# lppllppl920/EndoscopyDepthEstimation-Pytorch

Hardware: AMD Instinct MI355X
Metric: train frame-pairs/sec at 256x320 bs=8 (higher is better)
Workload: dtype f32

## Files before the change

endoscopydepthestimation-pytorch_amd/csrc/conv_dma_kernels.h:

```cpp
#pragma once

#include "conv_kernels.h"

namespace endo {

static __device__ __attribute__((aligned(16))) float g_pad_consts[8] = {__builtin_nanf(""), __builtin_nanf(""), __builtin_nanf(""), __builtin_nanf(""),
                                                                  0.0f, 0.0f, 0.0f, 0.0f};

typedef const __attribute__((address_space(1))) void* gptr_t;
typedef __attribute__((address_space(3))) void* lptr_t;

template <int KS, int KC, int Q, int WX, int R, int NBUF, int VEC, int IN = IN_PLAIN>
struct ConvDmaSmem {
    using G = ConvGeom<KS, KC, WX, R, VEC>;
    static constexpr int kW = KS * KS * KC * 16 * Q;
    static constexpr int kUG = (G::kTileX / 2) * (G::kTileY / 2);
    static constexpr int kUI = kUG / 4;
    static constexpr int kUStride = ((kUG + kUI - 8 + 31) / 32) * 32 + 8;
    static constexpr int kChan = (IN == IN_UNPOOL) ? kUStride : G::kCS;
    static constexpr int kBuf = KC * kChan + kW;
    static constexpr int kTail = 4 * 16 * Q + 8 * 16 * Q;
    static size_t bytes(int bn_cap) { return sizeof(float) * (NBUF * kBuf + 3 * bn_cap + kTail); }
};

template <int KS, int KC, int Q, int IN, int EPI, int WX, int R, int NBUF, int MINW, int VEC, int XF, int EXP = 0, int PH = -1, int BF = 0>
__global__ void __launch_bounds__(kConvThreads, MINW) conv_dma_kernel(const ConvParams p0) {
    static_assert(BF == 0 || (PH < 0 && (KS == 3 || KS == 1) && (IN == IN_BNRELU || IN == IN_PLAIN || (IN == IN_UNPOOL && KS == 1))),
                  "bf16 operands: the ordinary 3x3 convolution and the 1x1 convolutions of the transition-down layers");
    static_assert(PH < 0 || (KS == 3 && (Q % 2) == 0 && IN == IN_PLAIN && EPI == EPI_FWD), "phase mode is the transition-up forward");
    static_assert(IN != IN_UNPOOL || (KS == 1 && R % 2 == 0), "UNPOOL is the transition-down data gradient (1x1)");
    static_assert(NBUF == 1 || NBUF == 2, "one or two LDS buffers");
    static_assert(VEC == 1 || (VEC == 4 && IN != IN_UPSAMPLE && IN != IN_UNPOOL && IN != IN_SUBPIX), "16-byte DMA needs contiguous sources");
    static_assert(IN != IN_SUBPIX || (KS == 3 && EPI == EPI_FWD && PH < 0), "sub-pixel input mode is the transition-up data gradient");
    using G = ConvGeom<KS, KC, WX, R, VEC>;
    using S = ConvDmaSmem<KS, KC, Q, WX, R, NBUF, VEC, IN>;
    constexpr int KK = KS * KS;
    constexpr int NB = 16 * Q;
    constexpr int kWElems = S::kW;
    constexpr int kWPre = (kWElems + kConvThreads - 1) / kConvThreads;
    constexpr bool kDgrad = (EPI == EPI_DGRAD_BN || EPI == EPI_DGRAD_SUMPOOL);
    constexpr int kPhW = 2 * 12 * 16 + 16;
    static_assert(PH < 0 || KC * kPhW <= kWElems, "the phase weights fit the ordinary weight buffer");
    constexpr int kSubW = 4 * 16 * Q + 16;

    extern __shared__ __attribute__((aligned(16))) float smem[];
    float* s_aux = smem + NBUF * S::kBuf;
    int grp, n;
    group_of(p0, blockIdx.z, grp, n);
    const ConvParams p = group_view(p0, grp);
    const int groups = p0.group_n > 0 ? gridDim.z / p0.group_n : 1;
    const bool first_of_group = blockIdx.x == 0 && blockIdx.y == 0 && n == 0;
    (void)groups; (void)first_of_group;
    const int cap = p.bn_cap;

    const int tid = threadIdx.x;
    const int lane = tid & 63;
    const int wave = __builtin_amdgcn_readfirstlane(tid >> 6);
    const int tile = (gridDim.x & 7) == 0 ? xcd_remap(blockIdx.x, gridDim.x) : blockIdx.x;
    const int x0 = (tile % p.tiles_x) * G::kTileX;
    const int y0 = (tile / p.tiles_x) * G::kTileY;
    const int ph = PH == 2 ? static_cast<int>(blockIdx.y) : PH;
    const int co_base = (p.ksplit > 0 || PH == 2) ? 0 : blockIdx.y * NB;

    if constexpr (IN == IN_BNRELU) {
// ... 4 lines not shown
            s_aux[cap + c] = mean;
            s_aux[2 * cap + c] = beta;
        }
        for (int c = p.cin + tid; c < ((p.cin + KC - 1) / KC) * KC; c += kConvThreads) {
            s_aux[c] = 0.f; s_aux[cap + c] = 0.f; s_aux[2 * cap + c] = 0.f;
        }
    }
    if constexpr (EPI == EPI_DGRAD_BN) {
        float* cst = s_aux + 3 * cap;
        if (tid < NB) {
            const int c = co_base + tid;
            float mean = 0.f, rstd = 0.f, scale = 0.f, beta = 0.f;
            if (c < p.cout) {
                mean = p.bn_saved[2 * c];
                rstd = p.bn_saved[2 * c + 1];
                scale = p.bn_gamma[c] * rstd;
                beta = p.bn_beta[c];
            }
            cst[4 * tid] = scale; cst[4 * tid + 1] = beta; cst[4 * tid + 2] = mean; cst[4 * tid + 3] = rstd;
        }
    }

    f32x4 acc[R][Q];
#pragma unroll
    for (int r = 0; r < R; ++r)
#pragma unroll
        for (int q = 0; q < Q; ++q) acc[r][q] = f32x4{0.f, 0.f, 0.f, 0.f};

    const int wx = (wave % WX) * 16;
    const int wy = (wave / WX) * R;
    const int li = lane & 15;
    const int lk = lane >> 4;

    int goff[G::kPos];
    unsigned pos_ok = 0;
#pragma unroll
    for (int k = 0; k < G::kPos; ++k) {
        const int e = tid + k * kConvThreads;
        goff[k] = 0;
        if (e < G::kUnits) {
            const int ry = e / (G::kCols / VEC);
            const int rx = (e - ry * (G::kCols / VEC)) * VEC;
            const int gy = y0 - G::kHalo + ry;
            const int gx = x0 - G::kLeft + rx;
            if (gy >= 0 && gy < p.h && gx >= 0 && gx < p.w) {
                pos_ok |= (1u << k);
                if constexpr (IN == IN_UPSAMPLE) goff[k] = (gy >> 1) * p.in_w + (gx >> 1);
                else if constexpr (IN == IN_SUBPIX) goff[k] = 2 * gy * p.in_w + 2 * gx;
                else goff[k] = gy * p.in_w + gx;
            }
        }
    }
    constexpr int kUSlots = (IN == IN_UNPOOL) ? (KC * S::kUStride + kConvThreads - 1) / kConvThreads : 1;
    int uoff[kUSlots];
    if constexpr (IN == IN_UNPOOL) {
        constexpr int PC = G::kTileX / 2;
        const int ph = p.h >> 1, pw = p.w >> 1;
#pragma unroll
        for (int k = 0; k < kUSlots; ++k) {
            const int e = tid + k * kConvThreads;
            const int u = e % S::kUStride;
            int off = -1;
            if (e < KC * S::kUStride) {
                if (u < S::kUG) {
                    const int gy = (y0 >> 1) + u / PC, gx = (x0 >> 1) + u % PC;
                    if (gy < ph && gx < pw) off = gy * p.in_w + gx;
                } else if (u < S::kUG + S::kUI) {
                    const int q = u - S::kUG;
                    const int gy = (y0 >> 1) + q / (PC / 4), gx = (x0 >> 1) + 4 * (q % (PC / 4));
                    if (gy < ph && gx < pw) off = gy * p.in_w + gx;
                }
            }
            uoff[k] = off;
        }
    }
    const float* in_n = p.in + n * p.in_ns;
    const float* pad_in = g_pad_consts + (IN == IN_BNRELU ? 0 : 4);
    const float* pad_zero = g_pad_consts + 4;
    const int nchunks_all = (p.cin + KC - 1) / KC;
    int chunk_begin = 0, nchunks = nchunks_all;
    ConvParams po = p;
    if (p.ksplit > 0) {
        const int per = (nchunks_all + p.ksplit - 1) / p.ksplit;
        chunk_begin = blockIdx.y * per;
        nchunks = min(nchunks_all, chunk_begin + per);
        po.out = p.out + blockIdx.y * p.split_stride;
    }

    auto issue_dma = [&](int chunk, int buf) {
        const int c_base = chunk * KC;
        float* s_in = smem + buf * S::kBuf;
        float* s_w = s_in + KC * S::kChan;
        if constexpr (IN == IN_UNPOOL) {
            const uint8_t* idx_n = p.in_idx + n * p.idx_ns;
#pragma unroll
            for (int k = 0; k < kUSlots; ++k) {
                const int e0 = k * kConvThreads + wave * 64;
                if (e0 < KC * S::kUStride) {
                    const int e = e0 + lane;
                    const int ch = c_base + e / S::kUStride;
                    const bool is_code = (e % S::kUStride) >= S::kUG;
                    const void* src = pad_zero;
                    if (uoff[k] >= 0 && ch < p.cin) {
                        const int64_t o = static_cast<int64_t>(ch) * p.in_cs + uoff[k];
                        src = is_code ? static_cast<const void*>(idx_n + o) : static_cast<const void*>(in_n + o);
                    }
                    if (e < KC * S::kUStride) __builtin_amdgcn_global_load_lds((gptr_t)src, (lptr_t)(s_in + e0), 4, 0, 0);
                }
            }
        }
        int sub_ph = 0;
        if constexpr (IN == IN_SUBPIX) sub_ph = c_base / p.sub_c;
#pragma unroll
        for (int c = 0; c < (IN == IN_UNPOOL ? 0 : KC); ++c) {
            const int ch = c_base + c;
            const float* plane = in_n + static_cast<int64_t>(ch) * p.in_cs;
            if constexpr (IN == IN_SUBPIX)
                plane = in_n + static_cast<int64_t>(ch - sub_ph * p.sub_c) * p.in_cs + (sub_ph >> 1) * p.in_w + (sub_ph & 1);
#pragma unroll
            for (int k = 0; k < G::kPos; ++k) {
                const int e0 = k * kConvThreads + wave * 64;
                if (e0 < G::kUnits) {
                    const bool ok = (ch < p.cin) && (pos_ok & (1u << k));
                    const float* src = ok ? plane + goff[k] : pad_in;
                    if (e0 + lane < G::kUnits) {
// ... 203 lines not shown
                        const float* a_base = s_in + (quad * 4 + lk) * G::kCS + wy * G::kCols + wx + li + G::kColOff;
                        const float* b_base = s_w + (quad * 4 + lk) * NB + li;
                        float sc = 1.f, mn = 0.f, bt = 0.f;
                        if constexpr (IN == IN_BNRELU && !kInPlace) {
                            const int ch = chunk * KC + quad * 4 + lk;
                            sc = s_aux[ch]; mn = s_aux[cap + ch]; bt = s_aux[2 * cap + ch];
                        }
#pragma unroll
                        for (int r = 0; r < R; ++r) {
                            const float v = a_base[r * G::kCols];
                            a[i][r] = (IN == IN_BNRELU && !kInPlace) ? __builtin_fmaxf(fmaf(v - mn, sc, bt), 0.f) : v;
                        }
#pragma unroll
                        for (int q = 0; q < Q; ++q) b[i][q] = b_base[q * 16];
                    } else {
#pragma unroll
                        for (int r = 0; r < R; ++r) a[i][r] = 0.f;
#pragma unroll
                        for (int q = 0; q < Q; ++q) b[i][q] = 0.f;
                    }
                }
                bf16x4_bits ap[R];
#pragma unroll
                for (int r = 0; r < R; ++r) ap[r] = pack_bf16x4(a[0][r], a[1][r], a[2][r], a[3][r]);
#pragma unroll
                for (int q = 0; q < Q; ++q) {
                    const bf16x4_bits bp = pack_bf16x4(b[0][q], b[1][q], b[2][q], b[3][q]);
#pragma unroll
                    for (int r = 0; r < R; ++r) acc[r][q] = __builtin_amdgcn_mfma_f32_16x16x16bf16_1k(ap[r], bp, acc[r][q], 0, 0, 0);
                }
            }
            return;
        }
#pragma unroll
        for (int quad = 0; quad < KC / 4; ++quad) {
            const float* a_base = s_in + (quad * 4 + lk) * G::kCS + wy * G::kCols + wx + li + G::kColOff;
            const float* b_base = s_w + (quad * 4 + lk) * NB + li;
            float sc = 1.f, mn = 0.f, bt = 0.f;
            if constexpr (IN == IN_BNRELU && !kInPlace) {
                const int ch = chunk * KC + quad * 4 + lk;
                sc = s_aux[ch]; mn = s_aux[cap + ch]; bt = s_aux[2 * cap + ch];
            }
#pragma unroll
            for (int dx = 0; dx < KS; ++dx) {
                float a[R + KS - 1];
                if constexpr (BF != 0) {
#pragma unroll
                    for (int r = 0; r < R + 2; ++r) {
                        const float v = a_base[r * G::kCols + dx];
                        a[r] = (IN == IN_BNRELU && !kInPlace) ? __builtin_fmaxf(fmaf(v - mn, sc, bt), 0.f) : v;
                    }
                    bf16x4_bits ap[R];
#pragma unroll
                    for (int r = 0; r < R; ++r) ap[r] = pack_bf16x4(a[r], a[r + 1], a[r + 2], 0.f);
#pragma unroll
                    for (int q = 0; q < Q; ++q) {
                        const bf16x4_bits bp = pack_bf16x4(b_base[(0 * KS + dx) * KC * NB + q * 16], b_base[(1 * KS + dx) * KC * NB + q * 16],
                                                           b_base[(2 * KS + dx) * KC * NB + q * 16], 0.f);
#pragma unroll
                        for (int r = 0; r < R; ++r) acc[r][q] = __builtin_amdgcn_mfma_f32_16x16x16bf16_1k(ap[r], bp, acc[r][q], 0, 0, 0);
                    }
                    continue;
                }
                if constexpr (IN == IN_BNRELU && !kInPlace && !(EXP & 2)) {
                    typedef float f32x2 __attribute__((ext_vector_type(2)));
                    constexpr int NR = R + KS - 1;
// ... 27 lines not shown
                            const int tyi = dy - (sub_alpha == 0 ? 1 : 0), txi = dx - (sub_beta == 0 ? 1 : 0);
                            b = s_w[(quad * 4 + lk) * kSubW + (tyi * 2 + txi) * NB + q * 16 + li];
                        } else if constexpr (PH >= 0) {
                            const int slot = dx == 0 ? q : (dx == 1 ? Q / 2 + q : Q / 2 + Q + (q - Q / 2));
                            b = s_w[(quad * 4 + lk) * kPhW + ((dy - ph) * 2 * Q + slot) * 16 + li];
                        } else {
                            b = b_base[(dy * KS + dx) * KC * NB + q * 16];
                        }
#pragma unroll
                        for (int r = 0; r < R; ++r)
                            acc[r][q] = __builtin_amdgcn_mfma_f32_16x16x4f32(a[r + dy], b, acc[r][q], 0, 0, 0);
                    }
                }
            }
        }
    };

    issue_dma(chunk_begin, 0);
    if constexpr (kInPlace) {
        __syncthreads();
        asm volatile("s_waitcnt vmcnt(0)" ::: "memory");
        transform_own(chunk_begin, 0);
        __syncthreads();
        for (int chunk = chunk_begin; chunk < nchunks; ++chunk) {
            const int b = (chunk - chunk_begin) & 1;
            if (chunk + 1 < nchunks) issue_dma(chunk + 1, b ^ 1);
            compute(chunk, b);
            if (chunk + 1 < nchunks) {
                asm volatile("s_waitcnt vmcnt(0)" ::: "memory");
                transform_own(chunk + 1, b ^ 1);
            }
            __syncthreads();
        }
    } else {
        for (int chunk = chunk_begin; chunk < nchunks; ++chunk) {
            const int b = (chunk - chunk_begin) % NBUF;
            if (!(EXP & 4) || chunk == chunk_begin) asm volatile("s_waitcnt vmcnt(0)" ::: "memory");
            __syncthreads();
            if (NBUF == 2 && chunk + 1 < nchunks && !(EXP & 1)) issue_dma(chunk + 1, b ^ 1);
            compute(chunk, b);
            if (NBUF == 1 && chunk + 1 < nchunks) {
                __syncthreads();
                issue_dma(chunk + 1, 0);
            }
        }
    }

    if constexpr (EPI == EPI_DGRAD_BN) {
        if (use_pre) {
            const float* cst = s_aux + 3 * cap;
            float* s_red = s_aux + 3 * cap + 4 * NB;
            const int px = x0 + wx + 4 * lk;
#pragma unroll
            for (int q = 0; q < Q; ++q) {
                const int jloc = q * 16 + li;
                const int co = co_base + jloc;
                const float scale = cst[4 * jloc], beta = cst[4 * jloc + 1], mean = cst[4 * jloc + 2], rstd = cst[4 * jloc + 3];
                float s1 = 0.f, s2 = 0.f;
#pragma unroll
                for (int r = 0; r < R; ++r) {
                    const int y = y0 + wy + r;
                    if (co < p.cout && y < p.h && px + 3 < p.w) {
                        f32x4 o = dpre[r][q];
#pragma unroll
                        for (int e = 0; e < 4; ++e) {
                            const float xc = xpre[r][q][e] - mean;
// ... 107 lines not shown
```

endoscopydepthestimation-pytorch_amd/csrc/net.hip:

```cpp
#include <new>
#include <vector>

#include "dgrad_kernels.h"
#include "dgrad_block_kernels.h"
#include "dgrad_newmap_kernels.h"
#include "td_dgrad_kernels.h"
#include "td_fwd_kernels.h"
#include "wgrad_taps_kernels.h"
#include "wgrad1x1_kernels.h"
#include "wgrad_nsplit_kernels.h"
#include "wgrad_x3_kernels.h"
#include "wgrad_f34_kernels.h"
#include "wgrad_subpix_kernels.h"
#include "wino_fwd_kernels.h"
#include "wino4_fwd_kernels.h"
#include "dgrad_wino_kernels.h"
#include "dgrad_wino3_kernels.h"


namespace endo {

int run_dgrad_wino3_nl4(const DgradBlockParams& p, const float* const* u, hipStream_t stream);
bool dgrad_wino3p_applies(const DgradBlockParams& p);
int run_dgrad_wino3p_nl4(const DgradBlockParams& p, const float* const* u, int blocks, double* fw_parts, int* blocks_used, hipStream_t stream);
// ... 451 lines not shown
        const int stride = gridDim.y * blockDim.x * 4;
        for (int i = (blockIdx.y * blockDim.x + threadIdx.x) * 4; i < plane; i += stride) {
            const f32x4 gv = *reinterpret_cast<const f32x4*>(gp + i);
            const f32x4 pv = *reinterpret_cast<const f32x4*>(pp + i);
            f32x4 uv = {1.f, 1.f, 1.f, 1.f};
            if (c < cin) uv = *reinterpret_cast<const f32x4*>(up + i);
            part += gv[0] * sign_of(pv[0]) * uv[0] + gv[1] * sign_of(pv[1]) * uv[1];
            part2 += gv[2] * sign_of(pv[2]) * uv[2] + gv[3] * sign_of(pv[3]) * uv[3];
        }
    } else {
        for (int i = blockIdx.y * blockDim.x + threadIdx.x; i < plane; i += gridDim.y * blockDim.x)
            part += gp[i] * sign_of(pp[i]) * (c < cin ? up[i] : 1.f);
    }
    const int lane = threadIdx.x & 63, wave = threadIdx.x >> 6;
    double v = wave_sum(static_cast<double>(part + part2));
    if (lane == 0) scratch[wave] = v;
    __syncthreads();
    if (threadIdx.x == 0) {
        const float t = static_cast<float>(scratch[0] + scratch[1] + scratch[2] + scratch[3]);
        if (c < cin) atomicAdd(gw + c, t); else atomicAdd(gb, t);
    }
}

__global__ void __launch_bounds__(64) final_w_reduce_kernel(const double* __restrict__ parts, int nblocks, int count, float* __restrict__ gw) {
    const int c = blockIdx.x;
    double t = 0.0;
    for (int b = threadIdx.x; b < nblocks; b += 64) t += parts[static_cast<int64_t>(b) * count + c];
    t = wave_sum(t);
    if (threadIdx.x == 0) atomicAdd(gw + c, static_cast<float>(t));
}

constexpr int kBlocks = 2 * kLevels + 1, kDense = kBlocks * kLayers;

enum class DenseFwd { Wino4, Wino2_32x16, Wino2_32x8, SplitK, Direct32x8, Direct16x8, DirectAuto };
struct FwdPlan {
    struct Dense {
        DenseFwd form;
        int stages;
        int ksplit;
        bool chunk_weights;
    } dense[kDense];
    bool bf16;
    bool wino4_weights;
    bool fuse_final;
    bool td_persistent[kLevels];
    bool tu_subpix[kLevels];
};

enum class NewMap { Bf16, Persistent, Vec16, Dword };
enum class BasePass { Block8, Block8Bf16, Wino3, Wino3Persistent, Wino8 };
enum class DenseWgrad { F34, X3, NSplit, Taps, Direct };
enum class TdDgrad { Persistent, Runs128, Dma, Staged };
enum class TuWgrad { Subpix, Taps, Direct };
enum class TuDgrad { Subpix32x8, Subpix16x8, Subpix16x4, Plain };
enum class FirstWgrad { F34Prep, F34, Taps, Direct };
struct BwdPlan {
    struct Block {
        bool fused;
        NewMap newmap[kLayers];
        BasePass base;
        bool wino3_layout;
    } block[kBlocks];
    DenseWgrad wgrad[kDense];
    bool td_wgrad_dma[kLevels];
    TdDgrad td_dgrad[kLevels];
    TuWgrad tu_wgrad[kLevels];
    TuDgrad tu_dgrad[kLevels];
    int overlap;
    bool bf16_wgrad, bf16_dgrad;
    int f34_blocks;
    bool dgrad_weights;
    bool use_virt;
    bool virt_base;
// ... 60 lines not shown
    p.cin = cin;
}

static void fill_out(const Ctx& c, ConvParams& p, float* base, int level, int oc0, int cout) {
    const auto& lv = c.net->lv[level];
    p.out = base + oc0 * lv.plane;
    p.out_ns = lv.t * lv.plane;
    p.out_cs = static_cast<int>(lv.plane);
    p.out_w = lv.w;
    p.cout = cout;
}

static void fill_grid(const Ctx& c, ConvParams& p, int level) {
    const auto& lv = c.net->lv[level];
    p.n = c.nt(); p.h = lv.h; p.w = lv.w;
    p.group_n = c.net->n; p.gs = c.net->gs; p.in_gs = c.net->gs; p.out_gs = c.net->gs;
}

static double conv_flops(const endo_net* net, int level, int cin, int cout, int ks) {
    return 2.0 * net->n * net->groups * net->lv[level].plane * cin * cout * ks * ks;
}

static void default_options(int (&opt)[ENDO_OPT_COUNT]) {
    opt[ENDO_OPT_WINO_FWD] = 5;
    opt[ENDO_OPT_WINO_DGRAD] = 3;
    opt[ENDO_OPT_DGRAD_VEC] = 2;
    opt[ENDO_OPT_WINO_MIN_TILES] = 1024;
    opt[ENDO_OPT_MFMA_BF16] = 0;
    opt[ENDO_OPT_WGRAD_OVERLAP] = 1;
    opt[ENDO_OPT_MFMA_X3] = 0;
    opt[ENDO_OPT_WGRAD_F34] = 1;
    opt[ENDO_OPT_FINAL_VIRTUAL] = 1;
    opt[ENDO_OPT_TD_PERSIST] = 3;
}
static int bf16_mask(const int* opt) { const int v = opt[ENDO_OPT_MFMA_BF16]; return v == 1 ? 7 : (v >> 1); }

struct DenseBlock { int level, ic0, c0; const BnP* bn; const ConvP* cv; bool base_overwrite; };
static DenseBlock dense_block(int b) {
    const Table& tb = table();
    if (b < kLevels) return {b, 48, down_in(b), tb.down_bn[b], tb.down_conv[b], false};
    if (b == kLevels) return {kLevels, 0, 288, tb.bott_bn, tb.bott_conv, true};
    const int i = b - kLevels - 1, l = kLevels - 1 - i;
    return {l, 0, 96 + down_in(l), tb.up_bn[i], tb.up_conv[i], l > 0};
}
static long tile_count(const Ctx& c, int level, int tx, int ty) {
    const auto& lv = c.net->lv[level];
    return static_cast<long>((lv.w + tx - 1) / tx) * ((lv.h + ty - 1) / ty) * c.nt();
}

static ConvParams dense_fwd_params(const Ctx& c, const DenseBlock& k, int j, DenseFwd form) {
    const ConvP& cv = k.cv[j];
    const int oc0 = k.ic0 + k.c0 + kGrowth * j;
    ConvParams p{};
    fill_grid(c, p, k.level);
    fill_in(c, p, c.act(k.level), k.level, k.ic0, cv.cin);
    fill_bn_in(c, p, k.bn[j], k.level, k.ic0);
    p.wgt = c.params + cv.w; p.bias = c.params + cv.b; p.w_cout = cv.cout; p.w_cin = cv.cin;
    fill_out(c, p, c.act(k.level), k.level, oc0, cv.cout);
    p.out_sums = c.out_sums(k.level, oc0);
    if (form == DenseFwd::Wino4) p.wgt = c.tape + c.net->wino4_off + cv.u / kWinoUStride * kW4UStride;
    if (form == DenseFwd::Wino2_32x16 || form == DenseFwd::Wino2_32x8) p.wgt = c.tape + c.net->wino_off + cv.u;
    return p;
}

static ConvParams td_fwd_params(const Ctx& c, int level) {
    const BnP& b = table().td_bn[level];
    const ConvP& cv = table().td_conv[level];
    const int next = level + 1;
    const int oc0 = next < kLevels ? 48 : 0;
    ConvParams p{};
    fill_grid(c, p, level);
    fill_in(c, p, c.act(level), level, 48, cv.cin);
    fill_bn_in(c, p, b, level, 48);
    p.wgt = c.params + cv.w; p.bias = c.params + cv.b; p.w_cout = cv.cout; p.w_cin = cv.cin;
    fill_out(c, p, c.act(next), next, oc0, cv.cout);
    p.out_idx = c.idx(level);
    p.idx_ns = static_cast<int64_t>(cv.cout) * c.net->lv[next].plane;
    p.out_sums = c.out_sums(next, oc0);
    return p;
}

static FwdPlan plan_fwd(const Ctx& c) {
    const int* opt = c.net->opt;
    const int mode = opt[ENDO_OPT_WINO_FWD];
    const long min_tiles = opt[ENDO_OPT_WINO_MIN_TILES];
    FwdPlan pl{};
    pl.bf16 = (bf16_mask(opt) & 2) != 0;
    pl.wino4_weights = !pl.bf16 && mode == 5;
    for (int b = 0; b < kBlocks; ++b) {
        const DenseBlock k = dense_block(b);
        const long t64x16 = tile_count(c, k.level, 64, 16), t32x16 = tile_count(c, k.level, 32, 16), t32x8 = tile_count(c, k.level, 32, 8);
        const long t16x16 = tile_count(c, k.level, 16, 16), t16x8 = tile_count(c, k.level, 16, 8);
        const bool big = t32x16 >= min_tiles, small = t32x8 >= (min_tiles * 3) / 4;
        const bool wino4_tiles = mode == 5 && !pl.bf16 && 2 * t64x16 >= min_tiles;
        const bool wino2_tiles = mode != 0 && !pl.bf16 && (big || small);
        for (int j = 0; j < kLayers; ++j) {
            FwdPlan::Dense& d = pl.dense[b * kLayers + j];
            const int nchunks = (k.cv[j].cin + 15) / 16;
            d.chunk_weights = !pl.bf16 && !wino4_tiles && !wino2_tiles;
            d.stages = mode == 4 ? 4 : (mode == 3 ? 3 : 2);
            if (wino4_tiles && wino4_fwd_ok(dense_fwd_params(c, k, j, DenseFwd::Wino4))) {
                d.form = DenseFwd::Wino4;
            } else if (wino2_tiles && wino_fwd_ok(dense_fwd_params(c, k, j, DenseFwd::Wino2_32x16))) {
                d.form = big ? DenseFwd::Wino2_32x16 : DenseFwd::Wino2_32x8;
            } else if (t32x16 < 512 && t16x16 < 384 && t16x8 < 512 && nchunks >= 4) {
                int want = static_cast<int>(((t16x8 < 256 ? 512 : 768) + t16x8 - 1) / t16x8);
                if (want > nchunks) want = nchunks;
                const int per = (nchunks + want - 1) / want;
                d.form = DenseFwd::SplitK;
                d.ksplit = (nchunks + per - 1) / per;
            } else {
                d.form = (t32x16 < 1024 && t32x8 >= 1024) ? DenseFwd::Direct32x8
                       : (t32x16 < 1024 && t16x8 >= 768) ? DenseFwd::Direct16x8 : DenseFwd::DirectAuto;
            }
        }
    }
    pl.fuse_final = opt[ENDO_OPT_FINAL_VIRTUAL] && pl.dense[kDense - 1].form == DenseFwd::Wino4;
    for (int l = 0; l < kLevels; ++l) {
        pl.td_persistent[l] = (opt[ENDO_OPT_TD_PERSIST] & 2) && !pl.bf16 && c.training && td_fwd_ok(td_fwd_params(c, l));
        const ConvP& tu = table().tu_conv[kLevels - 1 - l];
        pl.tu_subpix[l] = c.net->lv[l + 1].w % 4 == 0 && tu.cout == kNew && tu.cin % 4 == 0;
    }
    return pl;
}

static int dense_fwd(const Ctx& c, int b, int j) {
    const DenseBlock k = dense_block(b);
    const FwdPlan::Dense& d = c.fwd->dense[b * kLayers + j];
    const ConvP& cv = k.cv[j];
    const auto& lv = c.net->lv[k.level];
    const int oc0 = k.ic0 + k.c0 + kGrowth * j;
    ConvParams p = dense_fwd_params(c, k, j, d.form);
    ProfScope prof(kProfConv3x3Dense, c.stream, conv_flops(c.net, k.level, cv.cin, cv.cout, 3),
                   4.0 * c.nt() * lv.plane * (cv.cin + cv.cout));
    const float* chunk_weights = d.chunk_weights ? c.tape + c.net->wino_off + cv.u : nullptr;
    const bool bf16 = c.fwd->bf16;
    switch (d.form) {
        case DenseFwd::Wino4:
            if (c.fwd->fuse_final && b == kBlocks - 1 && j == kLayers - 1) { p.fin_w = c.params + table().final_.w + k.ic0; p.fin_out = c.tape + c.net->pre_off; }
            return launch_wino4_fwd(p, c.stream);
        case DenseFwd::Wino2_32x16:
            return d.stages == 4 ? launch_wino_fwd<2, 4, 2, 4>(p, c.stream) : d.stages == 3 ? launch_wino_fwd<2, 4, 2, 3>(p, c.stream) : launch_wino_fwd<2, 4, 2, 2>(p, c.stream);
        case DenseFwd::Wino2_32x8:
            return d.stages == 4 ? launch_wino_fwd<1, 4, 3, 4>(p, c.stream) : d.stages == 3 ? launch_wino_fwd<1, 4, 3, 3>(p, c.stream) : launch_wino_fwd<1, 4, 3, 2>(p, c.stream);
        case DenseFwd::SplitK: {
            float* partial = c.tape + c.net->partial_off;
            p.ksplit = d.ksplit;
            p.split_stride = static_cast<int64_t>(c.net->n) * cv.cout * lv.plane;
            p.out = partial; p.out_ns = static_cast<int64_t>(cv.cout) * lv.plane;
            p.bias = nullptr; p.out_sums = nullptr;
            p.wgt_chunks = chunk_weights;
            int rc = bf16 ? launch_conv_dma<3, 16, 1, IN_BNRELU, EPI_FWD, 1, 2, 2, 1, 1>(p, c.stream)
                          : launch_conv_dma<3, 16, 1, IN_BNRELU, EPI_FWD, 1, 2, 2, 1>(p, c.stream);
            if (rc) return rc;
            int bx = static_cast<int>((lv.plane + 255) / 256);
            bx = bx > 8 ? 8 : bx;
            finalize_partial_kernel<<<dim3(bx, cv.cout, c.nt()), 256, 0, c.stream>>>(
                partial, p.split_stride, d.ksplit, p.out_ns, static_cast<int>(lv.plane), c.params + cv.b, c.act(k.level) + oc0 * lv.plane,
                lv.t * lv.plane, c.out_sums(k.level, oc0), c.net->n, c.net->gs);
            ENDO_LAUNCH_CHECK();
            return 0;
        }
        case DenseFwd::Direct32x8:
            return bf16 ? launch_conv_dma<3, 4, 1, IN_BNRELU, EPI_FWD, 2, 4, 2, 1, 1>(p, c.stream) : launch_conv_dma<3, 4, 1, IN_BNRELU, EPI_FWD, 2, 4, 2, 1>(p, c.stream);
        case DenseFwd::Direct16x8:
            return bf16 ? launch_conv_dma<3, 8, 1, IN_BNRELU, EPI_FWD, 1, 2, 2, 1, 1>(p, c.stream) : launch_conv_dma<3, 8, 1, IN_BNRELU, EPI_FWD, 1, 2, 2, 1>(p, c.stream);
        case DenseFwd::DirectAuto:
            if (bf16) return launch_conv_dma_auto<3, 4, 1, IN_BNRELU, EPI_FWD, 8, 2, 1, 1>(p, c.stream);
            p.wgt_chunks = chunk_weights;
            return launch_conv_dma_auto<3, 4, 1, IN_BNRELU, EPI_FWD, 8, 2, 1>(p, c.stream);
    }
    return ENDO_E_BADARG;
}

static int td_fwd(const Ctx& c, int level) {
    const ConvP& cv = table().td_conv[level];
    const ConvParams p = td_fwd_params(c, level);
    ProfScope prof(kProfConv1x1Pool, c.stream, conv_flops(c.net, level, cv.cin, cv.cout, 1),
                   4.0 * c.nt() * c.net->lv[level].plane * (cv.cin + cv.cout / 4.0));
    if (c.fwd->td_persistent[level]) return launch_td_fwd(p, device_cu_count(), c.stream);
    if (c.fwd->bf16) return launch_conv_dma_auto<1, 8, 3, IN_BNRELU, EPI_FWD_POOL, 4, 2, 1, 1>(p, c.stream);
    return launch_conv_dma_auto<1, 8, 3, IN_BNRELU, EPI_FWD_POOL, 4>(p, c.stream);
}

static int tu_fwd(const Ctx& c, int level, int src_level, int src_c0, const ConvP& cv) {
    ProfScope prof(kProfConv3x3Up, c.stream, conv_flops(c.net, level, cv.cin, cv.cout, 3),
                   4.0 * c.nt() * c.net->lv[level].plane * (cv.cin / 4.0 + cv.cout));
    if (c.fwd->tu_subpix[level]) {
        float* w3 = c.tape + c.net->partial_off;
        tu_phase_weights_kernel<<<(2 * cv.cin * 384 + 255) / 256, 256, 0, c.stream>>>(c.params + cv.w, cv.cout, cv.cin, w3);
        ENDO_LAUNCH_CHECK();
        ConvParams p{};
        fill_grid(c, p, src_level);
        fill_in(c, p, c.act(src_level), src_level, src_c0, cv.cin);
        p.wgt = w3; p.w_cout = 2 * cv.cout; p.w_cin = cv.cin;
// ... 567 lines not shown
    if (bn_index < 0 || bn_index >= static_cast<int>(tb.bn_order.size()) || which < 0 || which > 1) return -1;
    return tb.bn_order[bn_index]->run + which * tb.bn_order[bn_index]->c;
}
extern "C" int endo_net_level_channels(int level) { return (level < 0 || level > kLevels) ? -1 : level_channels(level); }
extern "C" int64_t endo_net_act_offset(const endo_net* net, int level) { return (!net || level < 0 || level > kLevels) ? -1 : net->lv[level].act; }

extern "C" int64_t endo_net_tape_offset(const endo_net* net, int what, int index) {
    if (!net) return -1;
    const Table& tb = table();
    switch (what) {
        case ENDO_TAPE_PRE: return net->pre_off;
        case ENDO_TAPE_BN_SAVED:
            if (index < 0 || index >= static_cast<int>(tb.bn_order.size())) return -1;
            return net->saved_off + 2 * tb.bn_order[index]->saved;
        case ENDO_TAPE_POOL:
            if (index < 0 || index >= kLevels) return -1;
            return net->idx_off[index];
        default: return -1;
    }
}

extern "C" int endo_net_fwd(endo_net* net, const float* params, float* bn_running, const float* x, float* out, float* tape,
                            int training, void* stream_) {
    if (!net || !params || !bn_running || !x || !out || !tape) return ENDO_E_BADARG;
    const Table& tb = table();
    Ctx c{net, params, bn_running, tape, nullptr, nullptr, training, static_cast<hipStream_t>(stream_)};
    const FwdPlan plan = plan_fwd(c);
    c.fwd = &plan;
    for (int g = 0; g < net->groups; ++g)
        ENDO_CHECK(hipMemsetAsync(reinterpret_cast<char*>(tape + g * net->gs) + net->sums_off, 0, net->sums_bytes, c.stream));
    if (!plan.bf16) {
        ProfScope prof(kProfSmall, c.stream, 0.0, 4.0 * (tb.wino_floats + tb.wino_floats * 9 / 16));
        WinoWeightTable wt = tb.wino;
        for (int l = 0; l < wt.layers; ++l) wt.mode[l] = plan.dense[l].chunk_weights ? 1 : 0;
        wino_fwd_weights_kernel<<<(wt.start[wt.layers] + 255) / 256, 256, 0, c.stream>>>(wt, params, tape + net->wino_off);
        ENDO_LAUNCH_CHECK();
        if (plan.wino4_weights) wino4_fwd_weights_kernel<<<(tb.wino4.start[tb.wino4.layers] + 255) / 256, 256, 0, c.stream>>>(tb.wino4, params, tape + net->wino4_off);
        ENDO_LAUNCH_CHECK();
    }
    int rc;
    {
        ConvParams p{};
        fill_grid(c, p, 0);
        p.in = x; p.in_ns = 3 * net->lv[0].plane; p.in_cs = static_cast<int>(net->lv[0].plane); p.in_w = net->w; p.cin = 3;
        p.in_gs = net->n * p.in_ns;
        p.wgt = params + tb.first.w; p.bias = params + tb.first.b; p.w_cout = kFirst; p.w_cin = 3;
        fill_out(c, p, c.act(0), 0, 48, kFirst);
        p.out_sums = c.out_sums(0, 48);
        ProfScope prof(kProfConvFirst, c.stream, conv_flops(net, 0, 3, kFirst, 3), 4.0 * c.nt() * net->lv[0].plane * (3 + kFirst));
        rc = launch_conv_dma_auto<3, 4, 3, IN_PLAIN, EPI_FWD>(p, c.stream);
        if (rc) return rc;
    }
    for (int b = 0; b < kBlocks; ++b) {
        if (b > kLevels) {
            const int i = b - kLevels - 1, l = kLevels - 1 - i;
            rc = tu_fwd(c, l, l + 1, (i == 0) ? 288 : 96 + down_in(l + 1), tb.tu_conv[i]);
            if (rc) return rc;
        }
        for (int j = 0; j < kLayers; ++j) {
            rc = dense_fwd(c, b, j);
            if (rc) return rc;
        }
        if (b < kLevels) {
            rc = td_fwd(c, b);
            if (rc) return rc;
        }
    }
// ... 118 lines not shown
```

endoscopydepthestimation-pytorch_amd/csrc/wino_fwd_kernels.h:

```cpp
#pragma once

#include "conv_dma_kernels.h"

namespace endo {

constexpr int kWinoUStride = 16 * 16 + 16;
constexpr int kWinoMaxLayers = 48;

struct WinoWeightTable {
    int layers;
    int start[kWinoMaxLayers + 1];
    int cin[kWinoMaxLayers];
    int cout[kWinoMaxLayers];
    int64_t w_off[kWinoMaxLayers];
    int64_t u_off[kWinoMaxLayers];
    int mode[kWinoMaxLayers];
};
constexpr int kDenseChunkFloats = 9 * 16 * 16;

__global__ void __launch_bounds__(256) wino_fwd_weights_kernel(const WinoWeightTable t, const float* __restrict__ params, float* __restrict__ u) {
    const int total = t.start[t.layers];
    for (int item = blockIdx.x * blockDim.x + threadIdx.x; item < total; item += gridDim.x * blockDim.x) {
        int l = 0;
        while (item >= t.start[l + 1]) ++l;
        const int e = item - t.start[l];
        const int ci = e >> 4, j = e & 15;
        float g[3][3];
#pragma unroll
        for (int a = 0; a < 3; ++a)
#pragma unroll
            for (int b = 0; b < 3; ++b) g[a][b] = 0.f;
        if (j < t.cout[l]) {
            const float* src = params + t.w_off[l] + (static_cast<int64_t>(j) * t.cin[l] + ci) * 9;
#pragma unroll
            for (int a = 0; a < 3; ++a)
#pragma unroll
                for (int b = 0; b < 3; ++b) g[a][b] = src[a * 3 + b];
        }
        if (t.mode[l] == 1) {
            float* dst = u + t.u_off[l] + static_cast<int64_t>(ci >> 4) * kDenseChunkFloats + (ci & 15) * 16 + j;
#pragma unroll
            for (int tap = 0; tap < 9; ++tap) dst[tap * 256] = g[tap / 3][tap % 3];
            if (ci == t.cin[l] - 1)
                for (int cz = (ci & 15) + 1; cz < 16; ++cz)
#pragma unroll
                    for (int tap = 0; tap < 9; ++tap) dst[tap * 256 + (cz - (ci & 15)) * 16] = 0.f;
            continue;
        }
        float h[4][3];
#pragma unroll
        for (int b = 0; b < 3; ++b) {
            h[0][b] = g[0][b];
            h[1][b] = 0.5f * (g[0][b] + g[1][b] + g[2][b]);
            h[2][b] = 0.5f * (g[0][b] - g[1][b] + g[2][b]);
            h[3][b] = g[2][b];
        }
        float* dst = u + t.u_off[l] + static_cast<int64_t>(ci) * kWinoUStride + j;
#pragma unroll
        for (int a = 0; a < 4; ++a) {
            dst[(4 * a + 0) * 16] = h[a][0];
            dst[(4 * a + 1) * 16] = 0.5f * (h[a][0] + h[a][1] + h[a][2]);
            dst[(4 * a + 2) * 16] = 0.5f * (h[a][0] - h[a][1] + h[a][2]);
            dst[(4 * a + 3) * 16] = h[a][2];
        }
        if (j == 0) {
#pragma unroll
            for (int k = 0; k < 16; ++k) dst[256 + k] = 0.f;
        }
    }
}

template <int R, int KC, int NS = 2>
struct WinoFwdGeom {
    static constexpr int kTileX = 32;
    static constexpr int kTileY = 8 * R;
    static constexpr int kLeft = 4;
    static constexpr int kCols = kTileX + 2 * kLeft;
    static constexpr int kRows = kTileY + 2;
    static constexpr int kPlane = kRows * kCols;
// ... 256 lines not shown
```

endoscopydepthestimation-pytorch_amd/models.py:

```python

import ctypes

import torch
from torch import nn

from . import _lib

GROWTH = 12
LAYERS = 4
FIRST = 48
LEVELS = 5


class ConvParams(nn.Module):

    def __init__(self, cin, cout, k):
        super().__init__()
        self.weight = nn.Parameter(torch.empty(cout, cin, k, k))
        self.bias = nn.Parameter(torch.zeros(cout))
        nn.init.kaiming_uniform_(self.weight, a=5 ** 0.5)


class FusedBatchNorm2d(nn.Module):

# ... 200 lines not shown
        if self._flat_grad is None or self._flat_grad.device != self._flat.device:
            if not create:
                return
            self._flat_grad_full = torch.zeros(self._flat.numel() + 1, dtype=torch.float32, device=self._flat.device)
            self._flat_grad = self._flat_grad_full[:self._flat.numel()]
            for p, off in zip(self._params, self._offsets):
                p.grad = self._flat_grad[off:off + p.numel()].view(p.shape)
            return
        base = self._flat_grad.data_ptr()
        intact = True
        for p, off in zip(self._params, self._offsets):
            g = p.grad
            if g is None or g.data_ptr() != base + 4 * off:
                intact = False
                break
        if not intact:
            self._flat_grad.zero_()
            for p, off in zip(self._params, self._offsets):
                p.grad = self._flat_grad[off:off + p.numel()].view(p.shape)

    def _handle(self, n, h, w, groups=1):
        key = (n, h, w, groups)
        if key not in self._handles:
            lib = _lib.load()
            if lib.endo_net_param_floats() != self._flat.numel():
                raise RuntimeError("parameter packing mismatch between Python and libendo_hip.so")
            hnd = ctypes.c_void_p()
            _lib.check(lib.endo_net_create_grouped(ctypes.byref(hnd), n, h, w, groups), "endo_net_create_grouped(%d,%d,%d,%d)" % key)
            for option_id, value in getattr(self, "_kernel_options", {}).items():
                lib.endo_net_set_option(hnd, option_id, value)
            self._handles[key] = (hnd, int(lib.endo_net_tape_floats(hnd)), int(lib.endo_net_gradws_floats(hnd)))
        return self._handles[key]

    _OPTION_DEFAULTS = {0: 5, 1: 3, 2: 2, 3: 1024, 4: 0, 5: 1, 6: 0, 7: 1, 8: 1, 9: 3}

    def set_kernel_option(self, option_id, value):
        option_id, value = int(option_id), int(value)
        if option_id not in self._OPTION_DEFAULTS:
            raise ValueError("unknown kernel option %d" % option_id)
        options = self.__dict__.setdefault("_kernel_options", {})
        old = options.get(option_id, self._OPTION_DEFAULTS[option_id])
        options[option_id] = value
        lib = _lib.load()
        for key, (hnd, _, _) in self._handles.items():
            if key[0] in ("bf16", "fp16"):
                continue
            rc = lib.endo_net_set_option(hnd, option_id, value)
            if rc < 0:
                raise RuntimeError("endo_net_set_option(%d, %d) failed: %d" % (option_id, value, rc))
        return old

    def kernel_option(self, option_id):
        return self.__dict__.get("_kernel_options", {}).get(int(option_id), self._OPTION_DEFAULTS[int(option_id)])

    def __del__(self):
        try:
            lib = _lib.load()
            for key, (hnd, _, _) in self._handles.items():
                {"bf16": lib.endo_net16_destroy, "fp16": lib.endo_net16h_destroy}.get(key[0], lib.endo_net_destroy)(hnd)
            self._handles = {}
        except Exception:
            pass

    def __getstate__(self):
        state = dict(self.__dict__)
        for key in ("_handles", "_gradws"):
            state[key] = {}
# ... 316 lines not shown
```

include/endo_hip.h:

```cpp
#ifndef ENDO_HIP_H
#define ENDO_HIP_H

#include <stdint.h>

#ifdef __cplusplus
extern "C" {
#endif

#define ENDO_E_BADARG (-1)
#define ENDO_E_UNSUPPORTED (-2)

#define ENDO_ABI_VERSION 6
int endo_abi_version(void);
const char* endo_error_string(int code);

int endo_depth_scale_fwd(const float* pred, const float* sparse_depth, const float* sparse_mask,
                         float* scaled, float* ratio, double* stats,
                         int n, int hw, float eps, void* stream);
int endo_depth_scale_bwd(const float* grad_scaled, const float* grad_ratio,
                         const float* pred, const float* sparse_depth, const double* stats,
                         float* grad_pred, double* work,
                         int n, int hw, float eps, void* stream);

int endo_flow_from_depth_fwd(const float* depth, const float* mask, const float* t, const float* R,
// ... 48 lines not shown
                   const float* sparse_flows_1, const float* sparse_flows_2,
                   const float* sparse_flow_masks_1, const float* sparse_flow_masks_2,
                   const float* t_1_wrt_2, const float* r_1_wrt_2, const float* t_2_wrt_1, const float* r_2_wrt_1,
                   const float* intrinsics, float sfl_weight, float dcl_weight, float eps,
                   float* losses, float* grad_pred_1, float* grad_pred_2, float* workspace,
                   int n, int h, int w, void* stream);
int endo_loss_head_planes(int n, int h, int w, int64_t* offsets);

int64_t endo_warp_consistency_workspace_floats(int n, int h, int w);
int64_t endo_warp_consistency_bytes(int n, int h, int w);
int endo_warp_consistency(const float* depth_1, const float* depth_2, const float* boundaries, const float* t_1_wrt_2,
                          const float* r_1_wrt_2, const float* t_2_wrt_1, const float* r_2_wrt_1, const float* intrinsics,
                          float dcl_weight, float eps, float* loss, float* grad_depth_1, float* grad_depth_2,
                          float* workspace, int n, int h, int w, void* stream);


int endo_mask_mul(const float* a, const float* mask, float* out, int n, int c, int hw, void* stream);

typedef struct endo_net endo_net;

int endo_net_create(endo_net** out, int n, int h, int w);
int endo_net_create_grouped(endo_net** out, int n, int h, int w, int groups);
int endo_net_groups(const endo_net* net);
#define ENDO_OPT_WINO_FWD 0
#define ENDO_OPT_WINO_DGRAD 1
#define ENDO_OPT_DGRAD_VEC 2
#define ENDO_OPT_WINO_MIN_TILES 3
#define ENDO_OPT_MFMA_BF16 4
#define ENDO_OPT_WGRAD_OVERLAP 5
#define ENDO_OPT_MFMA_X3 6
#define ENDO_OPT_WGRAD_F34 7
#define ENDO_OPT_FINAL_VIRTUAL 8
#define ENDO_OPT_TD_PERSIST 9
#define ENDO_OPT_COUNT 10
int endo_net_set_option(endo_net* net, int option_id, int value);
int endo_net_get_option(const endo_net* net, int option_id);
int64_t endo_net_group_stride(const endo_net* net);
void endo_net_destroy(endo_net* net);
int64_t endo_net_param_floats(void);
int64_t endo_net_bn_floats(void);
int64_t endo_net_tape_floats(const endo_net* net);
int64_t endo_net_gradws_floats(const endo_net* net);
int64_t endo_net_param_offset(int index);
int64_t endo_net_bn_offset(int bn_index, int which );

int endo_net_fwd(endo_net* net, const float* params, float* bn_running, const float* x, float* out,
                 float* tape, int training, void* stream);
int endo_net_bwd(endo_net* net, const float* params, const float* x, const float* tape,
                 const float* grad_out, float* grads, float* gradws, int training, void* stream);
int endo_net_level_channels(int level);
int64_t endo_net_act_offset(const endo_net* net, int level);
#define ENDO_TAPE_PRE 0
#define ENDO_TAPE_BN_SAVED 1
#define ENDO_TAPE_POOL 2
int64_t endo_net_tape_offset(const endo_net* net, int what, int index);

int endo_sgd_clip_step(float* params, float* grads, float* momentum, double* norm_out,
                       int64_t count, float lr, float mu, float max_norm, float grad_scale,
                       int first_step, const float* skip_flag, void* stream);

int endo_sparse_scatter(const double* points, int n_points, const double* projections, const double* extrinsics,
                        const float* visibility, const float* clean, const uint8_t* mask, int batch, int height, int width,
                        float depth_multiplier, int32_t* winner_scratch, float* depth_masks, float* depths, float* flow_masks,
                        float* flows, void* stream);

int endo_relative_poses(const double* pair_extrinsics, int batch, double scale,
                        float* r_1_wrt_2, float* t_1_wrt_2, float* r_2_wrt_1, float* t_2_wrt_1, void* stream);
// ... 93 lines not shown
```

Before: 514.4.

## Add multi-stage LDS ring pipeline for dense-layer forward direct convolutions

Adds a 3- or 4-stage LDS ring buffer mode to the DMA convolution kernel for the dense layers' BN-ReLU forward. Each wave issues its own per-channel loads and waits with a hand-computed vmcnt, which lets several chunks stay in flight behind one barrier per chunk. The inner loop double-buffers register loads against MFMA issue. A new option (default on) picks this ring form for split-K and small direct layers, using 8-channel chunk-ordered weights and a new weight-prep layout. The risks are more LDS use, which lowers occupancy, and fragile vmcnt bookkeeping.

```diff
diff --git a/endoscopydepthestimation-pytorch_amd/csrc/conv_dma_kernels.h b/endoscopydepthestimation-pytorch_amd/csrc/conv_dma_kernels.h
--- a/endoscopydepthestimation-pytorch_amd/csrc/conv_dma_kernels.h
+++ b/endoscopydepthestimation-pytorch_amd/csrc/conv_dma_kernels.h
@@ -23,13 +23,30 @@
     static size_t bytes(int bn_cap) { return sizeof(float) * (NBUF * kBuf + 3 * bn_cap + kTail); }
 };
 
+template <int KC, int UNITS, int UNITS_W>
+constexpr int ring_dma_count(int wave) {
+    int n = (KC / 4) * ((UNITS + 63) / 64);
+    for (int j = wave; j * 64 < UNITS_W; j += 4) ++n;
+    return n;
+}
+template <int K, int AHEAD>
+__device__ __forceinline__ void ring_wait(int ahead) {
+    static_assert(K * AHEAD <= 63, "vmcnt is a 6-bit counter");
+    if constexpr (AHEAD >= 2) { if (ahead >= 2) { asm volatile("s_waitcnt vmcnt(%0) lgkmcnt(0)" :: "n"(2 * K) : "memory"); return; } }
+    if constexpr (AHEAD >= 1) { if (ahead >= 1) { asm volatile("s_waitcnt vmcnt(%0) lgkmcnt(0)" :: "n"(K) : "memory"); return; } }
+    asm volatile("s_waitcnt vmcnt(0) lgkmcnt(0)" ::: "memory");
+}
+
 template <int KS, int KC, int Q, int IN, int EPI, int WX, int R, int NBUF, int MINW, int VEC, int XF, int EXP = 0, int PH = -1, int BF = 0>
 __global__ void __launch_bounds__(kConvThreads, MINW) conv_dma_kernel(const ConvParams p0) {
     static_assert(BF == 0 || (PH < 0 && (KS == 3 || KS == 1) && (IN == IN_BNRELU || IN == IN_PLAIN || (IN == IN_UNPOOL && KS == 1))),
                   "bf16 operands: the ordinary 3x3 convolution and the 1x1 convolutions of the transition-down layers");
     static_assert(PH < 0 || (KS == 3 && (Q % 2) == 0 && IN == IN_PLAIN && EPI == EPI_FWD), "phase mode is the transition-up forward");
     static_assert(IN != IN_UNPOOL || (KS == 1 && R % 2 == 0), "UNPOOL is the transition-down data gradient (1x1)");
-    static_assert(NBUF == 1 || NBUF == 2, "one or two LDS buffers");
+    constexpr bool kRing = NBUF >= 3;
+    static_assert(NBUF >= 1 && NBUF <= 4, "one or two LDS buffers, or a ring of three or four stages");
+    static_assert(!kRing || (KS == 3 && (KC == 8 || KC == 16) && Q == 1 && IN == IN_BNRELU && EPI == EPI_FWD && XF == 0 && EXP == 0 && PH < 0 && BF == 0),
+                  "the ring form is the dense layers' forward on prepared chunk-ordered weights");
     static_assert(VEC == 1 || (VEC == 4 && IN != IN_UPSAMPLE && IN != IN_UNPOOL && IN != IN_SUBPIX), "16-byte DMA needs contiguous sources");
     static_assert(IN != IN_SUBPIX || (KS == 3 && EPI == EPI_FWD && PH < 0), "sub-pixel input mode is the transition-up data gradient");
     using G = ConvGeom<KS, KC, WX, R, VEC>;
@@ -100,11 +117,12 @@
     const int li = lane & 15;
     const int lk = lane >> 4;
 
-    int goff[G::kPos];
+    constexpr int kPosN = kRing ? (G::kUnits + 63) / 64 : G::kPos;
+    int goff[kPosN];
     unsigned pos_ok = 0;
 #pragma unroll
-    for (int k = 0; k < G::kPos; ++k) {
-        const int e = tid + k * kConvThreads;
+    for (int k = 0; k < kPosN; ++k) {
+        const int e = kRing ? lane + k * 64 : tid + k * kConvThreads;
         goff[k] = 0;
         if (e < G::kUnits) {
             const int ry = e / (G::kCols / VEC);
@@ -149,7 +167,7 @@
     int chunk_begin = 0, nchunks = nchunks_all;
     ConvParams po = p;
     if (p.ksplit > 0) {
-        const int per = (nchunks_all + p.ksplit - 1) / p.ksplit;
+        const int per = kRing ? (((p.cin + 15) / 16 + p.ksplit - 1) / p.ksplit) * (16 / KC) : (nchunks_all + p.ksplit - 1) / p.ksplit;
         chunk_begin = blockIdx.y * per;
         nchunks = min(nchunks_all, chunk_begin + per);
         po.out = p.out + blockIdx.y * p.split_stride;
@@ -159,6 +177,32 @@
         const int c_base = chunk * KC;
         float* s_in = smem + buf * S::kBuf;
         float* s_w = s_in + KC * S::kChan;
+        if constexpr (kRing) {
+#pragma unroll
+            for (int i = 0; i < KC / 4; ++i) {
+                const int c = 4 * i + wave;
+                const int ch = c_base + c;
+                const float* plane = in_n + static_cast<int64_t>(ch) * p.in_cs;
+#pragma unroll
+                for (int k = 0; k < kPosN; ++k) {
+                    const bool ok = (ch < p.cin) && (pos_ok & (1u << k));
+                    const float* src = ok ? plane + goff[k] : pad_in;
+                    if (k * 64 + lane < G::kUnits) {
+                        if constexpr (VEC == 4) __builtin_amdgcn_global_load_lds((gptr_t)src, (lptr_t)(s_in + c * G::kCS + 256 * k), 16, 0, 0);
+                        else __builtin_amdgcn_global_load_lds((gptr_t)src, (lptr_t)(s_in + c * G::kCS + 64 * k), 4, 0, 0);
+                    }
+                }
+            }
+            constexpr int kUnitsW = kWElems / 4;
+            const float* wsrc = p.wgt_chunks + static_cast<int64_t>(chunk) * kWElems;
+#pragma unroll
+            for (int i = 0; i * 256 < kUnitsW; ++i) {
+                const int u0 = (4 * i + wave) * 64;
+                if (u0 < kUnitsW && u0 + lane < kUnitsW)
+                    __builtin_amdgcn_global_load_lds((gptr_t)(wsrc + 4 * (u0 + lane)), (lptr_t)(s_w + 4 * u0), 16, 0, 0);
+            }
+            return;
+        }
         if constexpr (IN == IN_UNPOOL) {
             const uint8_t* idx_n = p.in_idx + n * p.idx_ns;
 #pragma unroll
@@ -428,6 +472,42 @@
             }
             return;
         }
+        if constexpr (kRing) {
+            constexpr int NG = (KC / 4) * KS;
+            float araw[2][R + KS - 1], bv[2][KS], cst[2][3];
+            auto load = [&](int g, int slot) {
+                const int quad = g / KS, dx = g % KS;
+                const float* a_base = s_in + (quad * 4 + lk) * G::kCS + wy * G::kCols + wx + li + G::kColOff;
+                const float* b_base = s_w + (quad * 4 + lk) * NB + li;
+#pragma unroll
+                for (int r = 0; r < R + KS - 1; ++r) araw[slot][r] = a_base[r * G::kCols + dx];
+#pragma unroll
+                for (int dy = 0; dy < KS; ++dy) bv[slot][dy] = b_base[(dy * KS + dx) * KC * NB];
+                if (dx == 0) {
+                    const int ch = chunk * KC + quad * 4 + lk;
+                    cst[quad & 1][0] = s_aux[ch]; cst[quad & 1][1] = s_aux[cap + ch]; cst[quad & 1][2] = s_aux[2 * cap + ch];
+                }
+            };
+            load(0, 0);
+#pragma unroll
+            for (int g = 0; g < NG; ++g) {
+                const float sc = cst[(g / KS) & 1][0], mn = cst[(g / KS) & 1][1], bt = cst[(g / KS) & 1][2];
+                float a[R + KS - 1];
+#pragma unroll
+                for (int r = 0; r < R + KS - 1; ++r) a[r] = __builtin_fmaxf(fmaf(araw[g & 1][r] - mn, sc, bt), 0.f);
+#pragma unroll
+                for (int r = 0; r < R; ++r) acc[r][0] = __builtin_amdgcn_mfma_f32_16x16x4f32(a[r], bv[g & 1][0], acc[r][0], 0, 0, 0);
+                __builtin_amdgcn_sched_barrier(0);
+                if (g + 1 < NG) load(g + 1, (g + 1) & 1);
+                __builtin_amdgcn_sched_barrier(0);
+#pragma unroll
+                for (int dy = 1; dy < KS; ++dy)
+#pragma unroll
+                    for (int r = 0; r < R; ++r) acc[r][0] = __builtin_amdgcn_mfma_f32_16x16x4f32(a[r + dy], bv[g & 1][dy], acc[r][0], 0, 0, 0);
+                __builtin_amdgcn_sched_barrier(0);
+            }
+            return;
+        }
 #pragma unroll
         for (int quad = 0; quad < KC / 4; ++quad) {
             const float* a_base = s_in + (quad * 4 + lk) * G::kCS + wy * G::kCols + wx + li + G::kColOff;
@@ -521,6 +601,30 @@
             }
             __syncthreads();
         }
+    } else if constexpr (kRing) {
+        constexpr int AHEAD = NBUF - 2;
+        constexpr int kUW = kWElems / 4;
+        int fill = 0;
+#pragma unroll 1
+        for (int chunk = chunk_begin; chunk < nchunks && fill < NBUF - 1; ++chunk, ++fill) issue_dma(chunk, fill);
+        int b = 0;
+#pragma unroll 1
+        for (int chunk = chunk_begin; chunk < nchunks; ++chunk) {
+            const int left = nchunks - 1 - chunk;
+            const int ahead = left < AHEAD ? left : AHEAD;
+            switch (wave) {
+                case 0: ring_wait<ring_dma_count<KC, G::kUnits, kUW>(0), AHEAD>(ahead); break;
+                case 1: ring_wait<ring_dma_count<KC, G::kUnits, kUW>(1), AHEAD>(ahead); break;
+                case 2: ring_wait<ring_dma_count<KC, G::kUnits, kUW>(2), AHEAD>(ahead); break;
+                default: ring_wait<ring_dma_count<KC, G::kUnits, kUW>(3), AHEAD>(ahead); break;
+            }
+            __builtin_amdgcn_sched_barrier(0);
+            __builtin_amdgcn_s_barrier();
+            __builtin_amdgcn_sched_barrier(0);
+            if (chunk + NBUF - 1 < nchunks) issue_dma(chunk + NBUF - 1, b == 0 ? NBUF - 1 : b - 1);
+            compute(chunk, b);
+            b = b + 1 == NBUF ? 0 : b + 1;
+        }
     } else {
         for (int chunk = chunk_begin; chunk < nchunks; ++chunk) {
             const int b = (chunk - chunk_begin) % NBUF;
diff --git a/endoscopydepthestimation-pytorch_amd/csrc/net.hip b/endoscopydepthestimation-pytorch_amd/csrc/net.hip
--- a/endoscopydepthestimation-pytorch_amd/csrc/net.hip
+++ b/endoscopydepthestimation-pytorch_amd/csrc/net.hip
@@ -507,13 +507,14 @@
 
 constexpr int kBlocks = 2 * kLevels + 1, kDense = kBlocks * kLayers;
 
-enum class DenseFwd { Wino4, Wino2_32x16, Wino2_32x8, SplitK, Direct32x8, Direct16x8, DirectAuto };
+enum class DenseFwd { Wino4, Wino2_32x16, Wino2_32x8, SplitK, WholeK16x4, Direct32x8, Direct16x8, DirectAuto, Ring16x8 };
 struct FwdPlan {
     struct Dense {
         DenseFwd form;
         int stages;
         int ksplit;
-        bool chunk_weights;
+        int ring;
+        int chunk_weights;
     } dense[kDense];
     bool bf16;
     bool wino4_weights;
@@ -640,6 +641,7 @@
     opt[ENDO_OPT_WGRAD_F34] = 1;
     opt[ENDO_OPT_FINAL_VIRTUAL] = 1;
     opt[ENDO_OPT_TD_PERSIST] = 3;
+    opt[ENDO_OPT_COARSE_FWD] = 1;
 }
 static int bf16_mask(const int* opt) { const int v = opt[ENDO_OPT_MFMA_BF16]; return v == 1 ? 7 : (v >> 1); }
 
@@ -692,6 +694,7 @@
     const int* opt = c.net->opt;
     const int mode = opt[ENDO_OPT_WINO_FWD];
     const long min_tiles = opt[ENDO_OPT_WINO_MIN_TILES];
+    const int coarse = opt[ENDO_OPT_COARSE_FWD];
     FwdPlan pl{};
     pl.bf16 = (bf16_mask(opt) & 2) != 0;
     pl.wino4_weights = !pl.bf16 && mode == 5;
@@ -705,7 +708,8 @@
         for (int j = 0; j < kLayers; ++j) {
             FwdPlan::Dense& d = pl.dense[b * kLayers + j];
             const int nchunks = (k.cv[j].cin + 15) / 16;
-            d.chunk_weights = !pl.bf16 && !wino4_tiles && !wino2_tiles;
+            d.chunk_weights = (!pl.bf16 && !wino4_tiles && !wino2_tiles) ? 16 : 0;
+            d.ring = 2;
             d.stages = mode == 4 ? 4 : (mode == 3 ? 3 : 2);
             if (wino4_tiles && wino4_fwd_ok(dense_fwd_params(c, k, j, DenseFwd::Wino4))) {
                 d.form = DenseFwd::Wino4;
@@ -717,9 +721,25 @@
                 const int per = (nchunks + want - 1) / want;
                 d.form = DenseFwd::SplitK;
                 d.ksplit = (nchunks + per - 1) / per;
+                const bool whole_k = coarse == 2;
+                const bool ring = coarse == 3 || coarse == 4 || (coarse == 1 && t16x8 >= 64);
+                if (d.chunk_weights && whole_k) {
+                    d.form = DenseFwd::WholeK16x4;
+                    d.ksplit = 0;
+                    d.ring = 4;
+                } else if (d.chunk_weights && ring) {
+                    d.ring = coarse == 4 ? 3 : 4;
+                    d.chunk_weights = d.ring == 4 ? 8 : 16;
+                }
             } else {
                 d.form = (t32x16 < 1024 && t32x8 >= 1024) ? DenseFwd::Direct32x8
                        : (t32x16 < 1024 && t16x8 >= 768) ? DenseFwd::Direct16x8 : DenseFwd::DirectAuto;
+                const bool ring = coarse >= 1;
+                if (d.form == DenseFwd::DirectAuto && d.chunk_weights && t32x16 < 512 && t16x16 < 384 && ring) {
+                    d.form = DenseFwd::Ring16x8;
+                    d.ring = coarse == 4 ? 3 : 4;
+                    d.chunk_weights = d.ring == 4 ? 8 : 16;
+                }
             }
         }
     }
@@ -759,7 +779,9 @@
             p.bias = nullptr; p.out_sums = nullptr;
             p.wgt_chunks = chunk_weights;
             int rc = bf16 ? launch_conv_dma<3, 16, 1, IN_BNRELU, EPI_FWD, 1, 2, 2, 1, 1>(p, c.stream)
-                          : launch_conv_dma<3, 16, 1, IN_BNRELU, EPI_FWD, 1, 2, 2, 1>(p, c.stream);
+                   : d.ring == 4 ? launch_conv_dma<3, 8, 1, IN_BNRELU, EPI_FWD, 1, 2, 4, 1>(p, c.stream)
+                   : d.ring == 3 ? launch_conv_dma<3, 16, 1, IN_BNRELU, EPI_FWD, 1, 2, 3, 1>(p, c.stream)
+                                 : launch_conv_dma<3, 16, 1, IN_BNRELU, EPI_FWD, 1, 2, 2, 1>(p, c.stream);
             if (rc) return rc;
             int bx = static_cast<int>((lv.plane + 255) / 256);
             bx = bx > 8 ? 8 : bx;
@@ -769,6 +791,12 @@
             ENDO_LAUNCH_CHECK();
             return 0;
         }
+        case DenseFwd::WholeK16x4:
+            p.wgt_chunks = chunk_weights;
+            return launch_conv_dma<3, 16, 1, IN_BNRELU, EPI_FWD, 1, 1, 4, 1>(p, c.stream);
+        case DenseFwd::Ring16x8:
+            p.wgt_chunks = chunk_weights;
+            return d.ring == 4 ? launch_conv_dma<3, 8, 1, IN_BNRELU, EPI_FWD, 1, 2, 4, 1>(p, c.stream) : launch_conv_dma<3, 16, 1, IN_BNRELU, EPI_FWD, 1, 2, 3, 1>(p, c.stream);
         case DenseFwd::Direct32x8:
             return bf16 ? launch_conv_dma<3, 4, 1, IN_BNRELU, EPI_FWD, 2, 4, 2, 1, 1>(p, c.stream) : launch_conv_dma<3, 4, 1, IN_BNRELU, EPI_FWD, 2, 4, 2, 1>(p, c.stream);
         case DenseFwd::Direct16x8:
@@ -1402,7 +1430,7 @@
     if (!plan.bf16) {
         ProfScope prof(kProfSmall, c.stream, 0.0, 4.0 * (tb.wino_floats + tb.wino_floats * 9 / 16));
         WinoWeightTable wt = tb.wino;
-        for (int l = 0; l < wt.layers; ++l) wt.mode[l] = plan.dense[l].chunk_weights ? 1 : 0;
+        for (int l = 0; l < wt.layers; ++l) wt.mode[l] = plan.dense[l].chunk_weights == 16 ? 1 : plan.dense[l].chunk_weights == 8 ? 2 : 0;
         wino_fwd_weights_kernel<<<(wt.start[wt.layers] + 255) / 256, 256, 0, c.stream>>>(wt, params, tape + net->wino_off);
         ENDO_LAUNCH_CHECK();
         if (plan.wino4_weights) wino4_fwd_weights_kernel<<<(tb.wino4.start[tb.wino4.layers] + 255) / 256, 256, 0, c.stream>>>(tb.wino4, params, tape + net->wino4_off);
diff --git a/endoscopydepthestimation-pytorch_amd/csrc/wino_fwd_kernels.h b/endoscopydepthestimation-pytorch_amd/csrc/wino_fwd_kernels.h
--- a/endoscopydepthestimation-pytorch_amd/csrc/wino_fwd_kernels.h
+++ b/endoscopydepthestimation-pytorch_amd/csrc/wino_fwd_kernels.h
@@ -16,7 +16,6 @@
     int64_t u_off[kWinoMaxLayers];
     int mode[kWinoMaxLayers];
 };
-constexpr int kDenseChunkFloats = 9 * 16 * 16;
 
 __global__ void __launch_bounds__(256) wino_fwd_weights_kernel(const WinoWeightTable t, const float* __restrict__ params, float* __restrict__ u) {
     const int total = t.start[t.layers];
@@ -37,14 +36,15 @@
 #pragma unroll
                 for (int b = 0; b < 3; ++b) g[a][b] = src[a * 3 + b];
         }
-        if (t.mode[l] == 1) {
-            float* dst = u + t.u_off[l] + static_cast<int64_t>(ci >> 4) * kDenseChunkFloats + (ci & 15) * 16 + j;
-#pragma unroll
-            for (int tap = 0; tap < 9; ++tap) dst[tap * 256] = g[tap / 3][tap % 3];
+        if (t.mode[l] != 0) {
+            const int kc = t.mode[l] == 2 ? 8 : 16;
+            float* dst = u + t.u_off[l] + static_cast<int64_t>(ci / kc) * (9 * kc * 16) + (ci % kc) * 16 + j;
+#pragma unroll
+            for (int tap = 0; tap < 9; ++tap) dst[tap * kc * 16] = g[tap / 3][tap % 3];
             if (ci == t.cin[l] - 1)
-                for (int cz = (ci & 15) + 1; cz < 16; ++cz)
-#pragma unroll
-                    for (int tap = 0; tap < 9; ++tap) dst[tap * 256 + (cz - (ci & 15)) * 16] = 0.f;
+                for (int cz = (ci % kc) + 1; cz < kc; ++cz)
+#pragma unroll
+                    for (int tap = 0; tap < 9; ++tap) dst[tap * kc * 16 + (cz - (ci % kc)) * 16] = 0.f;
             continue;
         }
         float h[4][3];
diff --git a/endoscopydepthestimation-pytorch_amd/models.py b/endoscopydepthestimation-pytorch_amd/models.py
--- a/endoscopydepthestimation-pytorch_amd/models.py
+++ b/endoscopydepthestimation-pytorch_amd/models.py
@@ -256,7 +256,7 @@
             self._handles[key] = (hnd, int(lib.endo_net_tape_floats(hnd)), int(lib.endo_net_gradws_floats(hnd)))
         return self._handles[key]
 
-    _OPTION_DEFAULTS = {0: 5, 1: 3, 2: 2, 3: 1024, 4: 0, 5: 1, 6: 0, 7: 1, 8: 1, 9: 3}
+    _OPTION_DEFAULTS = {0: 5, 1: 3, 2: 2, 3: 1024, 4: 0, 5: 1, 6: 0, 7: 1, 8: 1, 9: 3, 10: 1}
 
     def set_kernel_option(self, option_id, value):
         option_id, value = int(option_id), int(value)
diff --git a/include/endo_hip.h b/include/endo_hip.h
--- a/include/endo_hip.h
+++ b/include/endo_hip.h
@@ -104,7 +104,8 @@
 #define ENDO_OPT_WGRAD_F34 7
 #define ENDO_OPT_FINAL_VIRTUAL 8
 #define ENDO_OPT_TD_PERSIST 9
-#define ENDO_OPT_COUNT 10
+#define ENDO_OPT_COARSE_FWD 10
+#define ENDO_OPT_COUNT 11
 int endo_net_set_option(endo_net* net, int option_id, int value);
 int endo_net_get_option(const endo_net* net, int option_id);
 int64_t endo_net_group_stride(const endo_net* net);
```

New measurement: 518.2 (median of 6 runs). No clear change (+0.7%).
